# Tani843/Mixed_Precision_Multigrid_Solvers_for_PDEs

Hardware: AMD Instinct MI355X
Metric: MDoF/s per V-cycle on 2D Poisson (higher is better)
Workload: dtype f64 (adaptive policy); 1 GPU; 2D Poisson 4097^2 adaptive fp32->fp64 (switch_threshold=1e-6), V(2,2) weighted-Jacobi omega=0.8, 11 levels, 1xMI355X; levels=11, cycle=V(2,2), smoother=jacobi, parallelism=1 GPU

## Files before the change

### include/mghip.h

```cpp
#ifndef MGHIP_H
#define MGHIP_H

#include <stdint.h>

#ifdef __cplusplus
extern "C" {
#endif

#define MG_OK 0
#define MG_ERR_INVALID_VALUE (-1)
#define MG_ERR_NO_DEVICE (-2)
#define MG_ERR_HIP (-3)
#define MG_ERR_STATE (-4)
#define MG_ERR_ALLOC (-5)

typedef enum { MG_F32 = 0, MG_F64 = 1 } mg_dtype;
typedef enum {
  MG_JACOBI = 0,
  MG_RBGS = 1,
  MG_LEXGS = 2
} mg_smoother_t;
typedef enum { MG_CYCLE_V = 0, MG_CYCLE_W = 1, MG_CYCLE_F = 2 } mg_cycle_t;
typedef enum {
  MG_PREC_DOUBLE = 0,
// ... 16 lines not shown
  double coarse_tol;
  int32_t coarse_maxit;
  int32_t precision;
  double switch_threshold;
  double memory_threshold_gb;
  int32_t adaptive_reference_rule;
  int32_t device;
  int32_t profile;
  int32_t colour_offset;
  int32_t fused;
  int32_t tail;
  int32_t fmg_cycles;
  int32_t speculate;
  int32_t coarse_direct;
  int32_t mixed_split;
} mg_config;

typedef struct mg_stats {
  double solve_seconds;
  double h2d_seconds;
  double d2h_seconds;
  double initial_residual;
  int32_t precision_switches;
  int32_t last_coarse_sweeps;
  int32_t switch_reason;
  double fp32_floor;
} mg_stats;

typedef struct mg_handle mg_handle;

// ... 196 lines not shown
```

### mixed_precision_multigrid_solvers_for_pdes_amd/_build.py

```python
import os
import shutil
import subprocess
from concurrent.futures import ThreadPoolExecutor

HERE = os.path.dirname(os.path.abspath(__file__))
CSRC = os.path.join(HERE, "csrc")
LIBDIR = os.path.join(HERE, "lib")
OBJDIR = os.path.join(LIBDIR, "obj")
LIBPATH = os.path.join(LIBDIR, "libmghip.so")
SOURCES = [os.path.join(CSRC, n) for n in ("mg_launch.hip", "mg_engine.hip", "mg_solve.hip", "mg_dev.hip", "mg_plan.hip", "mg_tail.hip", "mg_pcg.hip", "mg_heat.hip")]
HEADERS = [os.path.join(CSRC, n) for n in ("mg_kernels.hpp", "mg_rb_kernels.hpp", "mg_tail_kernels.hpp", "mg_host.hpp", "mg_launch.hpp", "mg_pcg_kernels.hpp",
                                               "mg_heat_kernels.hpp")] + \
          [os.path.join(os.path.dirname(HERE), "include", n) for n in ("mghip.h", "mghip_heat.h")]
DEPS = SOURCES + HEADERS
_HOST_UNIT = ("mg_rb_kernels.hpp", "mg_tail_kernels.hpp", "mg_pcg_kernels.hpp", "mg_heat_kernels.hpp")
NOT_INCLUDED = {"mg_launch.hip": ("mg_tail_kernels.hpp", "mg_pcg_kernels.hpp", "mg_heat_kernels.hpp"),
                "mg_engine.hip": _HOST_UNIT, "mg_solve.hip": _HOST_UNIT, "mg_dev.hip": _HOST_UNIT,
                "mg_tail.hip": ("mg_launch.hpp", "mg_pcg_kernels.hpp", "mg_heat_kernels.hpp"),
                "mg_pcg.hip": ("mg_rb_kernels.hpp", "mg_tail_kernels.hpp", "mg_heat_kernels.hpp"),
                "mg_heat.hip": ("mg_rb_kernels.hpp", "mg_tail_kernels.hpp", "mg_launch.hpp", "mg_pcg_kernels.hpp"),
                "mg_plan.hip": ("mg_kernels.hpp", "mg_rb_kernels.hpp", "mg_tail_kernels.hpp", "mg_host.hpp", "mg_launch.hpp",
                                "mg_pcg_kernels.hpp", "mg_heat_kernels.hpp", "mghip_heat.h")}
FLAGS = ["--offload-arch=gfx950", "-O3", "-std=c++17", "-fPIC", "-ffp-contract=off", "-Wall", "-Wno-unused-function"]


def extra_flags():
    return os.environ.get("MGHIP_EXTRA_FLAGS", "").split()


def hipcc_path():
    for cand in (os.environ.get("HIPCC"), "/opt/rocm/bin/hipcc", shutil.which("hipcc")):
        if cand and os.path.exists(cand):
            return cand
    raise RuntimeError("hipcc not found (set HIPCC or install ROCm under /opt/rocm)")


def source_hash():
# ... 84 lines not shown
```

### mixed_precision_multigrid_solvers_for_pdes_amd/_lib.py

```python
import ctypes as C
import os

import numpy as np

from . import _build

MG_OK = 0
MG_ERR_INVALID_VALUE, MG_ERR_NO_DEVICE, MG_ERR_HIP, MG_ERR_STATE, MG_ERR_ALLOC, MG_ERR_TIMEOUT = -1, -2, -3, -4, -5, -6
MG_PLAN_PHASES = 7
PLAN_PHASE_NAMES = ("legs", "halo_copy", "halo_exchange", "coarse_allgather", "replicated_engine", "allreduce", "other")


class PlanTimeout(RuntimeError):
    """mg_plan_wait gave up (MG_ERR_TIMEOUT): the queued device work is still queued, so the process must not
    synchronise on it again -- report and leave (distributed.bench_main does, with os._exit)."""
MG_F32, MG_F64 = 0, 1
MG_JACOBI, MG_RBGS, MG_LEXGS = 0, 1, 2
MG_CYCLE_V, MG_CYCLE_W, MG_CYCLE_F = 0, 1, 2
MG_PREC_DOUBLE, MG_PREC_SINGLE, MG_PREC_MIXED_LEVELS, MG_PREC_ADAPTIVE, MG_PREC_SINGLE_MANAGED, MG_PREC_DEFECT = 0, 1, 2, 3, 4, 5

CYCLES = {"V": MG_CYCLE_V, "W": MG_CYCLE_W, "F": MG_CYCLE_F}


class MgConfig(C.Structure):
    _fields_ = [
        ("nx", C.c_int32), ("ny", C.c_int32),
        ("x0", C.c_double), ("x1", C.c_double), ("y0", C.c_double), ("y1", C.c_double),
        ("coeff", C.c_double),
        ("max_levels", C.c_int32), ("cycle", C.c_int32), ("pre", C.c_int32), ("post", C.c_int32),
        ("smoother", C.c_int32),
        ("omega", C.c_double),
        ("coarse_tol", C.c_double), ("coarse_maxit", C.c_int32),
        ("precision", C.c_int32),
        ("switch_threshold", C.c_double), ("memory_threshold_gb", C.c_double),
        ("adaptive_reference_rule", C.c_int32),
        ("device", C.c_int32), ("profile", C.c_int32), ("colour_offset", C.c_int32), ("fused", C.c_int32),
        ("tail", C.c_int32), ("fmg_cycles", C.c_int32), ("speculate", C.c_int32), ("coarse_direct", C.c_int32),
        ("mixed_split", C.c_int32),
    ]


class MgStats(C.Structure):
    _fields_ = [
        ("solve_seconds", C.c_double), ("h2d_seconds", C.c_double), ("d2h_seconds", C.c_double),
        ("initial_residual", C.c_double),
        ("precision_switches", C.c_int32), ("last_coarse_sweeps", C.c_int32),
        ("switch_reason", C.c_int32), ("fp32_floor", C.c_double),
    ]


class MgPcgStats(C.Structure):
    _fields_ = [("solve_seconds", C.c_double), ("precond_seconds", C.c_double), ("initial_residual", C.c_double),
                ("true_residual", C.c_double), ("iterations", C.c_int32), ("status", C.c_int32)]
# ... 239 lines not shown
```

### mixed_precision_multigrid_solvers_for_pdes_amd/csrc/mg_engine.hip

```cpp
#include "mg_launch.hpp"

#include <cstring>

namespace mgh {

std::string& last_error() {
  thread_local std::string msg;
  return msg;
}

static int upload(std::string* err, void* dev, int ddt, int ld, const void* host, int hdt, int nx, int ny, void* staging,
           hipStream_t st) {
  if (ddt == hdt) {
    HIPC(err, hipMemcpy2DAsync(dev, (size_t)ld * esize(ddt), host, (size_t)ny * esize(hdt), (size_t)ny * esize(hdt), nx,
                               hipMemcpyHostToDevice, st));
  } else {
    const int lds = pitch_elems(hdt, ny);
    HIPC(err, hipMemcpy2DAsync(staging, (size_t)lds * esize(hdt), host, (size_t)ny * esize(hdt), (size_t)ny * esize(hdt),
                               nx, hipMemcpyHostToDevice, st));
    d_convert(hdt, ddt, staging, dev, nx, ny, lds, ld, st);
  }
  HIPC(err, hipStreamSynchronize(st));
  return MG_OK;
}
// ... 170 lines not shown
    h->tail_start = k;
    break;
  }
  h->tail_direct = false;
  h->tail_minv_sigma = -1.0;
  if (h->tail_start < 0) return MG_OK;
  h->tail_direct = want_direct(h);
  std::vector<int> ops;
  tail_schedule(h, h->tail_start, h->tail_start, 2, ops);
  h->tail_nops = (int)ops.size();
  HIPC(&h->err, hipMalloc((void**)&h->d_tail_ops, sizeof(int) * ops.size()));
  HIPC(&h->err, hipMemcpy(h->d_tail_ops, ops.data(), sizeof(int) * ops.size(), hipMemcpyHostToDevice));
  if (tail_set_attrs(kTailPoolLimit + 1024) != MG_OK) h->tail_start = -1;
  return MG_OK;
}
static int plan_tail(mg_handle* h) {
  int rc = plan_tail_lds(h);
  if (rc != MG_OK) return rc;
  rc = tail2_plan(h);
  if (rc == MG_OK && h->tail2_start >= 0) h->tail_direct = want_direct(h);
  return rc;
}

static int build_coarse_inverse(mg_handle* h) {
  const Level& v = h->lv[h->L() - 1];
  const int cnx = v.nx, cny = v.ny, my = cny - 2, n = (cnx - 2) * my;
  if (n < 1 || n > 64) return fail(&h->err, MG_ERR_INVALID_VALUE, "coarse_direct: the coarsest grid has more than 64 unknowns");
  std::vector<double> a((size_t)cnx * cny, 1.0);
  if (h->varcoef) {
    const int dt = h->grid_dtype;
    std::vector<unsigned char> buf((size_t)cnx * v.ld[dt] * esize(dt));
    HIPC(&h->err, hipMemcpyAsync(buf.data(), v.a[dt], buf.size(), hipMemcpyDeviceToHost, h->stream));
    HIPC(&h->err, hipStreamSynchronize(h->stream));
    for (int i = 0; i < cnx; ++i)
      for (int j = 0; j < cny; ++j)
// ... 41 lines not shown
    HIPC(&h->err, hipMemcpy(h->d_minv, inv.data(), sizeof(double) * inv.size(), hipMemcpyHostToDevice));
    h->minv_n = n;
  }
  h->tail_minv_sigma = h->sigma;
  return MG_OK;
}

static void extra_sweeps(mg_handle* h, Level& f, int dt, LegGeom& g, int extra) {
  for (; extra > 0; extra -= g.nsweep) {
    g.nsweep = std::min(2, extra);
    d_sweeps(h->cfg.smoother, dt, f.u[dt], f.rhs[dt], f.t[dt], g, h->stream);
    std::swap(f.u[dt], f.t[dt]);
  }
}

int cycle_fused(mg_handle* h, int l, bool zero_u, int part) {
  const int L = h->L();
  Level& f = h->lv[l];
  const int dt = h->level_dtype(l);
  const size_t bytes = (size_t)f.nx * f.ld[dt] * esize(dt);
  const bool tail2 = l == h->tail2_start, tail_lds = l == h->tail_start && h->tail2_start < 0;
  if ((tail2 || tail_lds) && h->cfg.tail != 0) {
    if (h->tail_direct && h->tail_minv_sigma != h->sigma) { const int rc = build_coarse_inverse(h); if (rc != MG_OK) return rc; }
    if (tail2) return tail2_launch(h, zero_u);
    launch_tail(h, zero_u);
    return MG_OK;
  }
  if (l == L - 1) {
    coarse_solve(h, l, zero_u);
    return MG_OK;
  }
  Level& c = h->lv[l + 1];
  const int dc = h->level_dtype(l + 1);
  const bool fine = (l == 0);
  const int sm = h->cfg.smoother;
  LegGeom g = leg_geom(h, l, dt, dc);
  if (part != kPartBack) {
    StageTimer tm(h, &f, 0);
    if (h->cfg.pre > 2 && zero_u) { (void)hipMemsetAsync(f.u[dt], 0, bytes, h->stream); zero_u = false; }
    extra_sweeps(h, f, dt, g, h->cfg.pre - 2);
    g.nsweep = std::min(2, h->cfg.pre);
    d_down(sm, dt, dc, f.u[dt], f.rhs[dt], f.t[dt], c.rhs[dc], g, zero_u, h->stream);
    std::swap(f.u[dt], f.t[dt]);
  }
  for (int k = 0, n = h->visits(l); k < n && part != kPartBack; ++k) {
// ... 509 lines not shown
  HIPC(&h->err, hipSetDevice(h->cfg.device));
  for (int k = 0; k < ncycles; ++k) {
    const int rc = run_cycle(h);
    if (rc != MG_OK) return fail(&h->err, rc, "cycle: unsupported precision combination");
  }
  HIPC(&h->err, hipGetLastError());
  return MG_OK;
}

int mg_time_op(mg_handle* h, int op, int level, int dtype, int reps, double* avg_ms) {
  if (!h || !avg_ms || reps < 1 || level < 0 || level >= h->L() || !valid_dtype(dtype))
    return fail(h ? &h->err : nullptr, MG_ERR_INVALID_VALUE, "mg_time_op: bad argument");
  HIPC(&h->err, hipSetDevice(h->cfg.device));
  Level& v = h->lv[level];
  const int dt = dtype;
  if (op != 6 && (!v.u[dt] || !v.rhs[dt])) return fail(&h->err, MG_ERR_STATE, "mg_time_op: level has no arrays of that dtype");
  if ((op == 0 || op == 10) && h->cfg.smoother != MG_JACOBI) return fail(&h->err, MG_ERR_STATE, "mg_time_op: jacobi needs a Jacobi-configured handle");
  if ((op == 0 || (op >= 7 && op <= 9)) && !v.t[dt]) return fail(&h->err, MG_ERR_STATE, "mg_time_op: no ping-pong buffer on this level");
  if ((op == 2 || op == 4 || op == 5 || op == 7 || op == 8) && (level >= h->L() - 1 || !v.r[dt])) return fail(&h->err, MG_ERR_STATE, "mg_time_op: no coarser level");
  static const int exp_nsweep = exp_env("MG_EXP_NSWEEP", 2);
  h->norm_partials = 0;
  if (level == 0 && (op == 0 || op == 1 || (op >= 5 && op <= 9) || op == 12 || op == 13)) h->iterate_zero = false;
  std::vector<void*> hbm_sets;
  struct FreeSets { std::vector<void*>& v; ~FreeSets() { for (void* p : v) (void)hipFree(p); } } free_sets{hbm_sets};
  int nsets = 0, set_idx = 0;
  if (op == 10 || op == 11) {
    const size_t bytes = (size_t)v.nx * v.ld[dt] * esize(dt);
    nsets = std::max<int>(3, (int)((768ull << 20) / (3 * bytes)) + 1);
    for (int k = 0; k < 3 * nsets; ++k) {
      void* p = nullptr;
      HIPC(&h->err, hipMalloc(&p, bytes));
// ... 28 lines not shown
                  std::swap(v.u[dt], v.t[dt]); } break;
        case 8: { Level& c = h->lv[level + 1]; const int dc = c.u[dt] ? dt : 1 - dt;
                  LegGeom g = leg_geom(h, level, dt, dc); g.nsweep = exp_nsweep;
                  if (d_up(h->cfg.smoother, dt, dc, h->grid_dtype, v.u[dt], v.rhs[dt], v.t[dt], c.u[dc], h->partials, g, level == 0, h->stream) < 0) return MG_ERR_INVALID_VALUE;
                  std::swap(v.u[dt], v.t[dt]); } break;
        case 9: { LegGeom g = leg_geom(h, level, dt, -1); g.nsweep = exp_nsweep;
                  d_sweeps(h->cfg.smoother, dt, v.u[dt], v.rhs[dt], v.t[dt], g, h->stream);
                  std::swap(v.u[dt], v.t[dt]); } break;
        case 12: case 13: {
                  const int phase0 = h->phase;
                  if (h->cfg.precision == MG_PREC_ADAPTIVE) h->phase = dt;
                  const bool ok = level == 0 && span_ok(h) && h->level_dtype(0) == dt;
                  const int rc2 = ok ? cycle_span(h, op == 12) : MG_ERR_INVALID_VALUE;
                  h->phase = phase0;
                  if (rc2 != MG_OK) return rc2; } break;
        default: return MG_ERR_INVALID_VALUE;
      }
    }
    return MG_OK;
  };
  int rc = run(1);
  if (rc != MG_OK) { (void)hipEventDestroy(e0); (void)hipEventDestroy(e1); return fail(&h->err, rc, "mg_time_op: unsupported op"); }
  HIPC(&h->err, hipEventRecord(e0, h->stream));
  rc = run(reps);
  HIPC(&h->err, hipEventRecord(e1, h->stream));
  HIPC(&h->err, hipEventSynchronize(e1));
  float ms = 0;
  HIPC(&h->err, hipEventElapsedTime(&ms, e0, e1));
  (void)hipEventDestroy(e0); (void)hipEventDestroy(e1);
  *avg_ms = (double)ms / reps;
// ... 10 lines not shown
```

### mixed_precision_multigrid_solvers_for_pdes_amd/csrc/mg_host.hpp

```cpp
#pragma once

#include <hip/hip_runtime.h>

#include <algorithm>
#include <chrono>
#include <cmath>
#include <cstdlib>
#include <string>
#include <type_traits>
#include <vector>

#include "../../include/mghip.h"
#include "../../include/mghip_heat.h"
#include "mg_kernels.hpp"

namespace mgh {

std::string& last_error();
inline int fail(std::string* where, int code, const std::string& msg) {
  last_error() = msg;
  if (where) *where = msg;
  return code;
}
#define HIPC(errstr, call)                                                                         \
// ... 103 lines not shown
  bool have_rhs = false;
  bool varcoef = false;
  double sigma = 0.0;
  double rd_sigma = -1.0;
  double ring_sumsq[2] = {0, 0};
  unsigned rhs_gen = 1;
  unsigned rings_gen[2] = {0, 0};
  bool iterate_zero = false;
  unsigned zero_norm_gen[2] = {0, 0};
  double zero_norm_val[2] = {0, 0};
  int norm_partials = 0;
  int tail_start = -1;
  bool span_ring[2] = {false, false};
  int tail2_start = -1;
  int tail2_ntop = 0;
  int* d_tail_ops = nullptr;
  int tail_nops = 0;
  bool tail_direct = false;
  double tail_minv[81] = {0};
  double* d_minv = nullptr;
  int minv_n = 0;
  double tail_minv_sigma = -1.0;
  std::string err;
  std::vector<double> adapt_hist;

  int L() const { return (int)lv.size(); }
  int visits(int l) const {
    return cfg.cycle == MG_CYCLE_W ? 2 : cfg.cycle == MG_CYCLE_F ? std::max(1, 1 << std::max(0, L() - l - 2)) : 1;
  }
  int level_dtype_in(int l, int ph) const {
// ... 46 lines not shown
```

### mixed_precision_multigrid_solvers_for_pdes_amd/csrc/mg_launch.hpp

```cpp
#pragma once

#include "mg_host.hpp"

namespace mgh {

int pitch_elems(int dt, int ny);
size_t max_partials(int nx, int ny);

void d_jacobi(int dt, const void* u, const void* rhs, void* out, int nx, int ny, int ld, double hx, double hy,
              double omega, hipStream_t st, bool fine = false, double sigma = 0.0);
void d_rbgs_colour(int dt, void* u, const void* rhs, int nx, int ny, int ld, double hx, double hy, double omega,
                   int colour, int poff, hipStream_t st, bool fine = false, double sigma = 0.0);
void d_residual(int dt, const void* u, const void* f, void* r, int nx, int ny, int ld, double hx, double hy,
                double coeff, hipStream_t st, bool fine = false, double sigma = 0.0);
int d_residual_norm(int dt, const void* u, const void* f, double* partials, int nx, int ny, int ld, double hx,
                    double hy, double coeff, hipStream_t st, bool fine = false, double sigma = 0.0);
int d_sumsq(int dt, const void* x, double* partials, int ld, int i_lo, int i_hi, int j_lo, int j_hi, hipStream_t st);
void launch_reduce(const double* partials, int n, double* out, hipStream_t st, mg::HostMailbox* mailbox = nullptr,
                   unsigned long long seq = 0);
void d_restrict_sub(int di, int dout, const void* fine, void* coarse, int ldf, int nxc, int nyc, int ldc, int sides,
                    hipStream_t st);
void d_restrict(int di, int dout, const void* fine, void* coarse, int nxf, int nyf, int ldf, int ldc, hipStream_t st);
int d_prolong_sub(bool add, int dc, int df, int dcomp, const void* e, void* u, int nxf, int nyf, int ldf, int nxc, int nyc,
                  int ldc, int sides, hipStream_t st);
// ... 24 lines not shown
  double sigma = 0.0;
  const void* acoef = nullptr;
  const void* rdiag = nullptr;
  int rb = 0;
};
bool use_rb(const LegGeom& g);

int d_span(int dt, int dcomp, const void* u, const void* rhs, void* out_mid, void* out_next, const void* e_c, void* rhs_c,
           double* partials, const LegGeom& g, int nsweep_pre, hipStream_t st, int sm = MG_JACOBI);
void d_down(int sm, int dt, int dx, const void* u, const void* rhs, void* out, void* rhs_c, const LegGeom& g, bool zero_init,
            hipStream_t st);
int d_up(int sm, int dt, int dx, int dcomp, const void* u, const void* rhs, void* out, const void* e_c, double* partials,
         const LegGeom& g, bool norm, hipStream_t st);
void d_sweeps(int sm, int dt, const void* u, const void* rhs, void* out, const LegGeom& g, hipStream_t st);

constexpr size_t kTailPoolLimit = 150 * 1024;
size_t tail_pool_bytes(const mg_handle* h, int k, size_t esz, size_t esz_last);
int tail_set_attrs(size_t bytes);
void launch_tail(mg_handle* h, bool zero_top);

int launch_defect(mg_handle* h, bool update);
void d_stream_triad(int dt, const void* a, const void* b, void* out, int nx, int ny, int ld, hipStream_t st);
void d_residual_f32in_f64out(const float* u, const float* f, double* r, int nx, int ny, int ld_in, int ld_out, double hx,
                             double hy, double coeff, hipStream_t st);

}
```

### mixed_precision_multigrid_solvers_for_pdes_amd/engine.py

```python
import ctypes as C

import numpy as np

from . import _lib


def _direct_code(coarse_direct):
    import os
    if coarse_direct is None:
        coarse_direct = {"0": False, "1": True}.get(os.environ.get("MG_COARSE_DIRECT", "auto"), "auto")
    if isinstance(coarse_direct, str):
        if coarse_direct != "auto":
            raise ValueError(f"coarse_direct: True, False, 'auto' or None, not {coarse_direct!r}")
        return -1
    return int(bool(coarse_direct))


class MultigridEngine:

    def __init__(self, nx, ny, domain=(0.0, 1.0, 0.0, 1.0), coeff=-1.0, max_levels=4, cycle="V", pre=2, post=2,
                 smoother=_lib.MG_JACOBI, omega=0.8, coarse_tol=1e-12, coarse_maxit=1000,
                 precision=_lib.MG_PREC_DOUBLE, switch_threshold=1e-6, memory_threshold_gb=4.0,
                 adaptive_reference_rule=False, device=0, profile=False, colour_offset=0, fused=2, tail=True, speculate=True, fmg_cycles=0,
                 mixed_split=0, coarse_direct=None):
        lib = _lib.load()
        if isinstance(cycle, str):
            if cycle not in _lib.CYCLES:
                raise ValueError(f"unknown cycle type {cycle!r}")
            cycle = _lib.CYCLES[cycle]
        cfg = _lib.MgConfig(int(nx), int(ny), float(domain[0]), float(domain[1]), float(domain[2]), float(domain[3]),
                            float(coeff), int(max_levels), int(cycle), int(pre), int(post), int(smoother),
                            float(omega), float(coarse_tol), int(coarse_maxit), int(precision),
                            float(switch_threshold), float(memory_threshold_gb), int(bool(adaptive_reference_rule)),
                            int(device), int(bool(profile)), int(colour_offset), int(fused), int(tail), int(fmg_cycles), (2 if speculate is True else int(speculate)),
                            _direct_code(coarse_direct), int(mixed_split))
        self.cfg = cfg
        self._h = C.c_void_p(None)
        _lib.check(lib.mg_create(C.byref(cfg), C.byref(self._h)))
        self._lib = lib
        n = C.c_int(0)
        self._check(lib.mg_num_levels(self._h, C.byref(n)))
        self.num_levels = n.value
        self.shapes = []
        for l in range(self.num_levels):
            a, b = C.c_int(0), C.c_int(0)
            self._check(lib.mg_level_shape(self._h, l, C.byref(a), C.byref(b)))
            self.shapes.append((a.value, b.value))
        self.nx, self.ny = int(nx), int(ny)

    def _check(self, rc):
# ... 122 lines not shown
        self._check(self._lib.mg_get_solution_device(self._h, *self._dev_args(t)))

    def set_stream(self, stream):
        if stream is None:
            self._check(self._lib.mg_set_stream(self._h, None, 1))
        else:
            self._check(self._lib.mg_set_stream(self._h, stream if isinstance(stream, C.c_void_p) else C.c_void_p(int(stream)), 0))

    def get_stream(self):
        out = C.c_void_p(None)
        self._check(self._lib.mg_get_stream(self._h, C.byref(out)))
        return out.value or 0

    def time_op(self, op, level=0, dtype=np.float64, reps=20):
        ops = {"jacobi": 0, "rbgs": 1, "residual": 2, "residual_norm": 3, "restrict": 4, "prolong": 5, "cycle": 6,
               "down_leg": 7, "up_leg": 8, "sweeps2": 9, "jacobi_hbm": 10, "stream_hbm": 11, "span_leg": 12, "span_leg_nomid": 13}
        out = C.c_double(0.0)
        self._check(self._lib.mg_time_op(self._h, ops[op] if isinstance(op, str) else int(op), int(level),
                                         _lib.dtype_code(dtype), int(reps), C.byref(out)))
        return out.value

    def level_timings(self):
        res = {}
        for l in range(self.num_levels):
            t = (C.c_double * 3)()
            self._check(self._lib.mg_level_timings(self._h, l, t))
            res[l] = {"smooth_time": t[0], "restrict_time": t[1], "prolong_time": t[2]}
        return res
```

Measured before the change: 81550 MDoF/s.

## Merge two or three mid-size multigrid levels into single down and up kernels

Adds merged down and up kernels that process a group of up to three mid-size levels (at most 520 per side, just above the LDS tail) in one launch each. Each block keeps an overlapping halo region in LDS and runs the smoothing sweeps, residual and full-weighting restriction through all grouped levels, then on the way up does prolongation plus post-smoothing. This is meant to cut kernel launches and the global-memory round trips between levels. The cost is redundant halo computation and large LDS use at 512 threads per block, which may limit occupancy. It is enabled by default through MG_MERGE=1 for V-cycle Jacobi.

```diff
diff --git a/include/mghip.h b/include/mghip.h
--- a/include/mghip.h
+++ b/include/mghip.h
@@ -54,6 +54,7 @@
   int32_t speculate;
   int32_t coarse_direct;
   int32_t mixed_split;
+  int32_t merge;
 } mg_config;
 
 typedef struct mg_stats {
diff --git a/mixed_precision_multigrid_solvers_for_pdes_amd/_build.py b/mixed_precision_multigrid_solvers_for_pdes_amd/_build.py
--- a/mixed_precision_multigrid_solvers_for_pdes_amd/_build.py
+++ b/mixed_precision_multigrid_solvers_for_pdes_amd/_build.py
@@ -8,19 +8,21 @@
 LIBDIR = os.path.join(HERE, "lib")
 OBJDIR = os.path.join(LIBDIR, "obj")
 LIBPATH = os.path.join(LIBDIR, "libmghip.so")
-SOURCES = [os.path.join(CSRC, n) for n in ("mg_launch.hip", "mg_engine.hip", "mg_solve.hip", "mg_dev.hip", "mg_plan.hip", "mg_tail.hip", "mg_pcg.hip", "mg_heat.hip")]
+SOURCES = [os.path.join(CSRC, n) for n in ("mg_launch.hip", "mg_engine.hip", "mg_solve.hip", "mg_dev.hip", "mg_plan.hip", "mg_tail.hip", "mg_pcg.hip", "mg_heat.hip", "mg_merge.hip")]
 HEADERS = [os.path.join(CSRC, n) for n in ("mg_kernels.hpp", "mg_rb_kernels.hpp", "mg_tail_kernels.hpp", "mg_host.hpp", "mg_launch.hpp", "mg_pcg_kernels.hpp",
-                                               "mg_heat_kernels.hpp")] + \
+                                               "mg_heat_kernels.hpp", "mg_merge_kernels.hpp", "mg_merge_geom.hpp")] + \
           [os.path.join(os.path.dirname(HERE), "include", n) for n in ("mghip.h", "mghip_heat.h")]
 DEPS = SOURCES + HEADERS
-_HOST_UNIT = ("mg_rb_kernels.hpp", "mg_tail_kernels.hpp", "mg_pcg_kernels.hpp", "mg_heat_kernels.hpp")
-NOT_INCLUDED = {"mg_launch.hip": ("mg_tail_kernels.hpp", "mg_pcg_kernels.hpp", "mg_heat_kernels.hpp"),
+_MERGE = ("mg_merge_kernels.hpp", "mg_merge_geom.hpp")
+_HOST_UNIT = ("mg_rb_kernels.hpp", "mg_tail_kernels.hpp", "mg_pcg_kernels.hpp", "mg_heat_kernels.hpp") + _MERGE
+NOT_INCLUDED = {"mg_launch.hip": ("mg_tail_kernels.hpp", "mg_pcg_kernels.hpp", "mg_heat_kernels.hpp") + _MERGE,
+                "mg_merge.hip": ("mg_rb_kernels.hpp", "mg_tail_kernels.hpp", "mg_pcg_kernels.hpp", "mg_heat_kernels.hpp"),
                 "mg_engine.hip": _HOST_UNIT, "mg_solve.hip": _HOST_UNIT, "mg_dev.hip": _HOST_UNIT,
-                "mg_tail.hip": ("mg_launch.hpp", "mg_pcg_kernels.hpp", "mg_heat_kernels.hpp"),
-                "mg_pcg.hip": ("mg_rb_kernels.hpp", "mg_tail_kernels.hpp", "mg_heat_kernels.hpp"),
-                "mg_heat.hip": ("mg_rb_kernels.hpp", "mg_tail_kernels.hpp", "mg_launch.hpp", "mg_pcg_kernels.hpp"),
+                "mg_tail.hip": ("mg_launch.hpp", "mg_pcg_kernels.hpp", "mg_heat_kernels.hpp") + _MERGE,
+                "mg_pcg.hip": ("mg_rb_kernels.hpp", "mg_tail_kernels.hpp", "mg_heat_kernels.hpp") + _MERGE,
+                "mg_heat.hip": ("mg_rb_kernels.hpp", "mg_tail_kernels.hpp", "mg_launch.hpp", "mg_pcg_kernels.hpp") + _MERGE,
                 "mg_plan.hip": ("mg_kernels.hpp", "mg_rb_kernels.hpp", "mg_tail_kernels.hpp", "mg_host.hpp", "mg_launch.hpp",
-                                "mg_pcg_kernels.hpp", "mg_heat_kernels.hpp", "mghip_heat.h")}
+                                "mg_pcg_kernels.hpp", "mg_heat_kernels.hpp", "mghip_heat.h") + _MERGE}
 FLAGS = ["--offload-arch=gfx950", "-O3", "-std=c++17", "-fPIC", "-ffp-contract=off", "-Wall", "-Wno-unused-function"]
 
 
diff --git a/mixed_precision_multigrid_solvers_for_pdes_amd/_lib.py b/mixed_precision_multigrid_solvers_for_pdes_amd/_lib.py
--- a/mixed_precision_multigrid_solvers_for_pdes_amd/_lib.py
+++ b/mixed_precision_multigrid_solvers_for_pdes_amd/_lib.py
@@ -36,7 +36,7 @@
         ("adaptive_reference_rule", C.c_int32),
         ("device", C.c_int32), ("profile", C.c_int32), ("colour_offset", C.c_int32), ("fused", C.c_int32),
         ("tail", C.c_int32), ("fmg_cycles", C.c_int32), ("speculate", C.c_int32), ("coarse_direct", C.c_int32),
-        ("mixed_split", C.c_int32),
+        ("mixed_split", C.c_int32), ("merge", C.c_int32),
     ]
 
 
diff --git a/mixed_precision_multigrid_solvers_for_pdes_amd/csrc/mg_engine.hip b/mixed_precision_multigrid_solvers_for_pdes_amd/csrc/mg_engine.hip
--- a/mixed_precision_multigrid_solvers_for_pdes_amd/csrc/mg_engine.hip
+++ b/mixed_precision_multigrid_solvers_for_pdes_amd/csrc/mg_engine.hip
@@ -208,11 +208,25 @@
   if (tail_set_attrs(kTailPoolLimit + 1024) != MG_OK) h->tail_start = -1;
   return MG_OK;
 }
+static void plan_merge(mg_handle* h) {
+  h->merge_l0 = -1;
+  h->merge_nl = 0;
+  const int tail = h->tail2_start >= 0 ? h->tail2_start : h->tail_start;
+  if (tail < 0) return;
+  int first = tail;
+  while (first > 1 && std::max(h->lv[first - 1].nx, h->lv[first - 1].ny) <= 520) --first;
+  static const int max_nl = exp_env("MG_EXP_MERGE_NL", 3);
+  const int nl = std::min(std::min(3, max_nl), tail - first);
+  if (nl < 2) return;
+  h->merge_l0 = tail - nl;
+  h->merge_nl = nl;
+}
 static int plan_tail(mg_handle* h) {
   int rc = plan_tail_lds(h);
   if (rc != MG_OK) return rc;
   rc = tail2_plan(h);
   if (rc == MG_OK && h->tail2_start >= 0) h->tail_direct = want_direct(h);
+  plan_merge(h);
   return rc;
 }
 
@@ -284,6 +298,53 @@
   }
 }
 
+static MergeDesc merge_desc(const mg_handle* h, int dt, int nsweep) {
+  MergeDesc m;
+  m.nl = h->merge_nl;
+  for (int k = 0; k < m.nl; ++k) {
+    const Level& v = h->lv[h->merge_l0 + k];
+    MergeLevelDesc& d = m.lv[k];
+    d.u_in = v.u[dt]; d.u_out = v.t[dt]; d.rhs = v.rhs[dt];
+    d.nx = v.nx; d.ny = v.ny; d.ld = v.ld[dt]; d.hx = v.hx; d.hy = v.hy;
+  }
+  m.ldc = h->lv[h->merge_l0 + m.nl].ld[dt];
+  m.nsweep = nsweep; m.omega = h->cfg.omega; m.coeff = h->cfg.coeff; m.sigma = h->sigma;
+  return m;
+}
+static bool merge_arrays(const mg_handle* h, int dt) {
+  if (h->merge_l0 < 0) return false;
+  for (int l = h->merge_l0; l < h->merge_l0 + h->merge_nl; ++l)
+    if (!h->lv[l].u[dt] || !h->lv[l].t[dt] || !h->lv[l].rhs[dt]) return false;
+  const Level& c = h->lv[h->merge_l0 + h->merge_nl];
+  return c.u[dt] && c.rhs[dt];
+}
+static bool merge_ok(const mg_handle* h, int l, bool zero_u, int part) {
+  if (h->cfg.merge != 1 || l != h->merge_l0 || !zero_u || part != kPartFull || h->cfg.tail == 0) return false;
+  if (h->cfg.cycle != MG_CYCLE_V || h->cfg.smoother != MG_JACOBI || h->varcoef || h->cfg.profile) return false;
+  if (h->cfg.pre < 1 || h->cfg.pre > 2 || h->cfg.post < 1 || h->cfg.post > 2) return false;
+  const int dt = h->level_dtype(l);
+  for (int k = 1; k <= h->merge_nl; ++k)
+    if (h->level_dtype(l + k) != dt) return false;
+  if (dt == MG_F64 && h->grid_dtype == MG_F32) return false;
+  return merge_arrays(h, dt);
+}
+static void merge_swap(mg_handle* h, int dt) {
+  for (int l = h->merge_l0; l < h->merge_l0 + h->merge_nl; ++l) std::swap(h->lv[l].u[dt], h->lv[l].t[dt]);
+}
+static void down_merged(mg_handle* h, int dt, int nsweep) {
+  MergeDesc m = merge_desc(h, dt, nsweep);
+  m.coarse = h->lv[h->merge_l0 + h->merge_nl].rhs[dt];
+  d_down_merged(dt, m, h->stream);
+  merge_swap(h, dt);
+}
+static int up_merged(mg_handle* h, int dt, int nsweep) {
+  MergeDesc m = merge_desc(h, dt, nsweep);
+  m.coarse = h->lv[h->merge_l0 + h->merge_nl].u[dt];
+  if (d_up_merged(dt, h->grid_dtype, m, h->stream) < 0) return MG_ERR_INVALID_VALUE;
+  merge_swap(h, dt);
+  return MG_OK;
+}
+
 int cycle_fused(mg_handle* h, int l, bool zero_u, int part) {
   const int L = h->L();
   Level& f = h->lv[l];
@@ -299,6 +360,11 @@
   if (l == L - 1) {
     coarse_solve(h, l, zero_u);
     return MG_OK;
+  }
+  if (merge_ok(h, l, zero_u, part)) {
+    down_merged(h, dt, h->cfg.pre);
+    const int rc = cycle_fused(h, l + h->merge_nl, true);
+    return rc != MG_OK ? rc : up_merged(h, dt, h->cfg.post);
   }
   Level& c = h->lv[l + 1];
   const int dc = h->level_dtype(l + 1);
@@ -838,7 +904,10 @@
   HIPC(&h->err, hipSetDevice(h->cfg.device));
   Level& v = h->lv[level];
   const int dt = dtype;
-  if (op != 6 && (!v.u[dt] || !v.rhs[dt])) return fail(&h->err, MG_ERR_STATE, "mg_time_op: level has no arrays of that dtype");
+  if ((op == 14 || op == 15) && (!merge_arrays(h, dt) || level < h->merge_l0 || level >= h->merge_l0 + h->merge_nl || h->varcoef ||
+                                 (dt == MG_F64 && h->grid_dtype == MG_F32)))
+    return fail(&h->err, MG_ERR_STATE, "mg_time_op: no merged legs here (the level is in no group of levels, or not in that dtype)");
+  if (op != 6 && op != 14 && op != 15 && (!v.u[dt] || !v.rhs[dt])) return fail(&h->err, MG_ERR_STATE, "mg_time_op: level has no arrays of that dtype");
   if ((op == 0 || op == 10) && h->cfg.smoother != MG_JACOBI) return fail(&h->err, MG_ERR_STATE, "mg_time_op: jacobi needs a Jacobi-configured handle");
   if ((op == 0 || (op >= 7 && op <= 9)) && !v.t[dt]) return fail(&h->err, MG_ERR_STATE, "mg_time_op: no ping-pong buffer on this level");
   if ((op == 2 || op == 4 || op == 5 || op == 7 || op == 8) && (level >= h->L() - 1 || !v.r[dt])) return fail(&h->err, MG_ERR_STATE, "mg_time_op: no coarser level");
@@ -897,6 +966,8 @@
                   const int rc2 = ok ? cycle_span(h, op == 12) : MG_ERR_INVALID_VALUE;
                   h->phase = phase0;
                   if (rc2 != MG_OK) return rc2; } break;
+        case 14: down_merged(h, dt, exp_nsweep); break;
+        case 15: { const int rc2 = up_merged(h, dt, exp_nsweep); if (rc2 != MG_OK) return rc2; } break;
         default: return MG_ERR_INVALID_VALUE;
       }
     }
diff --git a/mixed_precision_multigrid_solvers_for_pdes_amd/csrc/mg_host.hpp b/mixed_precision_multigrid_solvers_for_pdes_amd/csrc/mg_host.hpp
--- a/mixed_precision_multigrid_solvers_for_pdes_amd/csrc/mg_host.hpp
+++ b/mixed_precision_multigrid_solvers_for_pdes_amd/csrc/mg_host.hpp
@@ -141,6 +141,8 @@
   bool span_ring[2] = {false, false};
   int tail2_start = -1;
   int tail2_ntop = 0;
+  int merge_l0 = -1;
+  int merge_nl = 0;
   int* d_tail_ops = nullptr;
   int tail_nops = 0;
   bool tail_direct = false;
diff --git a/mixed_precision_multigrid_solvers_for_pdes_amd/csrc/mg_launch.hpp b/mixed_precision_multigrid_solvers_for_pdes_amd/csrc/mg_launch.hpp
--- a/mixed_precision_multigrid_solvers_for_pdes_amd/csrc/mg_launch.hpp
+++ b/mixed_precision_multigrid_solvers_for_pdes_amd/csrc/mg_launch.hpp
@@ -62,6 +62,23 @@
          const LegGeom& g, bool norm, hipStream_t st);
 void d_sweeps(int sm, int dt, const void* u, const void* rhs, void* out, const LegGeom& g, hipStream_t st);
 
+struct MergeLevelDesc {
+  const void* u_in = nullptr;
+  void* u_out = nullptr;
+  void* rhs = nullptr;
+  int nx = 0, ny = 0, ld = 0;
+  double hx = 0, hy = 0;
+};
+struct MergeDesc {
+  MergeLevelDesc lv[3];
+  int nl = 0;
+  void* coarse = nullptr;
+  int ldc = 0, nsweep = 0;
+  double omega = 0, coeff = 0, sigma = 0;
+};
+void d_down_merged(int dt, const MergeDesc& m, hipStream_t st);
+int d_up_merged(int dt, int dcomp, const MergeDesc& m, hipStream_t st);
+
 constexpr size_t kTailPoolLimit = 150 * 1024;
 size_t tail_pool_bytes(const mg_handle* h, int k, size_t esz, size_t esz_last);
 int tail_set_attrs(size_t bytes);
diff --git a/mixed_precision_multigrid_solvers_for_pdes_amd/csrc/mg_merge.hip b/mixed_precision_multigrid_solvers_for_pdes_amd/csrc/mg_merge.hip
--- /dev/null
+++ b/mixed_precision_multigrid_solvers_for_pdes_amd/csrc/mg_merge.hip
@@ -0,0 +1,83 @@
+#include "mg_launch.hpp"
+#include "mg_merge_kernels.hpp"
+
+namespace mgh {
+
+constexpr int kDownBI = 4, kDownBJ = 4;
+constexpr int kUpBI = 32, kUpBJ = 32;
+
+template <typename T>
+static mg::MergeArgs<T> merge_args(const MergeDesc& m) {
+  mg::MergeArgs<T> a;
+  for (int k = 0; k < m.nl; ++k) {
+    const MergeLevelDesc& d = m.lv[k];
+    const Coef c = coefs(d.hx, d.hy, m.sigma);
+    mg::MergeLevel<T>& L = a.lv[k];
+    L.u_in = (const T*)d.u_in; L.u_out = (T*)d.u_out; L.rhs = (T*)d.rhs;
+    L.nx = d.nx; L.ny = d.ny; L.ld = d.ld; L.use_div = c.pow2 ? 0 : 1;
+    L.ihx2 = (T)c.ihx2; L.ihy2 = (T)c.ihy2; L.invD = (T)c.invD; L.D = (T)c.diag;
+  }
+  for (int k = m.nl; k < mgm::kMaxNL; ++k) a.lv[k] = a.lv[m.nl - 1];
+  a.coarse = (T*)m.coarse; a.ldc = m.ldc; a.nsweep = m.nsweep; a.nbj = 0;
+  a.omega = (T)m.omega; a.one_m_omega = (T)(1.0 - m.omega); a.coeff = (T)m.coeff;
+  return a;
+}
+
+template <typename T, int NL, int BI, int BJ>
+static void launch_down(const MergeDesc& m, hipStream_t st) {
+  mg::MergeArgs<T> a = merge_args<T>(m);
+  const int nbi = mgm::blocks(mgm::level_n(m.lv[0].nx, NL), BI);
+  a.nbj = mgm::blocks(mgm::level_n(m.lv[0].ny, NL), BJ);
+  hipLaunchKernelGGL((mg::merged_down_kernel<T, NL, BI, BJ>), dim3(nbi * a.nbj), dim3(mgm::kBlock), 0, st, a);
+}
+template <typename T, typename TC, int NL, int BI, int BJ>
+static void launch_up(const MergeDesc& m, hipStream_t st) {
+  mg::MergeArgs<T> a = merge_args<T>(m);
+  const int nbi = mgm::blocks(m.lv[0].nx, BI);
+  a.nbj = mgm::blocks(m.lv[0].ny, BJ);
+  hipLaunchKernelGGL((mg::merged_up_kernel<T, TC, NL, BI, BJ>), dim3(nbi * a.nbj), dim3(mgm::kBlock), 0, st, a);
+}
+
+template <typename T, int NL>
+static void down_shaped(const MergeDesc& m, hipStream_t st) {
+#ifdef MG_EXPERIMENTS
+  static const int shape = exp_env("MG_EXP_MERGE_DOWN", 0);
+  if (shape == 1) return launch_down<T, NL, 8, 8>(m, st);
+  if (shape == 2) return launch_down<T, NL, 4, 16>(m, st);
+  if (shape == 3) return launch_down<T, NL, 4, 8>(m, st);
+  if (shape == 4) return launch_down<T, NL, 2, 8>(m, st);
+#endif
+  launch_down<T, NL, kDownBI, kDownBJ>(m, st);
+}
+template <typename T, typename TC, int NL>
+static void up_shaped(const MergeDesc& m, hipStream_t st) {
+#ifdef MG_EXPERIMENTS
+  static const int shape = exp_env("MG_EXP_MERGE_UP", 0);
+  if (shape == 1) return launch_up<T, TC, NL, 64, 64>(m, st);
+  if (shape == 2) return launch_up<T, TC, NL, 32, 64>(m, st);
+  if (shape == 3) return launch_up<T, TC, NL, 16, 64>(m, st);
+  if (shape == 4) return launch_up<T, TC, NL, 16, 32>(m, st);
+#endif
+  launch_up<T, TC, NL, kUpBI, kUpBJ>(m, st);
+}
+
+void d_down_merged(int dt, const MergeDesc& m, hipStream_t st) {
+  with_dtype(dt, [&](auto t) {
+    using T = decltype(t);
+    if (m.nl == 3) down_shaped<T, 3>(m, st);
+    else down_shaped<T, 2>(m, st);
+  });
+}
+int d_up_merged(int dt, int dcomp, const MergeDesc& m, hipStream_t st) {
+  return with_dtype(dt, dcomp, [&](auto t, auto tc) {
+    using T = decltype(t); using TC = decltype(tc);
+    if constexpr (!interp_ok<T, T, TC>) return -1;
+    else {
+      if (m.nl == 3) up_shaped<T, TC, 3>(m, st);
+      else up_shaped<T, TC, 2>(m, st);
+      return 0;
+    }
+  });
+}
+
+}
diff --git a/mixed_precision_multigrid_solvers_for_pdes_amd/csrc/mg_merge_geom.hpp b/mixed_precision_multigrid_solvers_for_pdes_amd/csrc/mg_merge_geom.hpp
--- /dev/null
+++ b/mixed_precision_multigrid_solvers_for_pdes_amd/csrc/mg_merge_geom.hpp
@@ -0,0 +1,132 @@
+#pragma once
+
+#if defined(__HIPCC__)
+#define MGM_HD __host__ __device__ __forceinline__
+#else
+#define MGM_HD inline
+#endif
+
+namespace mgm {
+
+constexpr int kMaxNL = 3;
+constexpr int kMaxSweeps = 2;
+constexpr int kBlock = 512;
+constexpr int kLdsLimit = 160 * 1024;
+
+struct Iv { int lo, hi; };
+struct Box { Iv i, j; };
+
+MGM_HD int imin(int a, int b) { return a < b ? a : b; }
+MGM_HD int imax(int a, int b) { return a > b ? a : b; }
+MGM_HD int size(Iv a) { return a.hi > a.lo ? a.hi - a.lo : 0; }
+MGM_HD Iv grow(Iv a, int k) { return Iv{a.lo - k, a.hi + k}; }
+MGM_HD Iv interior(Iv a, int n) { return Iv{imax(a.lo, 1), imin(a.hi, n - 1)}; }
+MGM_HD bool has(Iv a, int x) { return x >= a.lo && x < a.hi; }
+MGM_HD bool has(const Box& b, int i, int j) { return has(b.i, i) && has(b.j, j); }
+MGM_HD bool inside(Iv in, Iv out) { return size(in) == 0 || (in.lo >= out.lo && in.hi <= out.hi); }
+MGM_HD int level_n(int n0, int k) { return ((n0 - 1) >> k) + 1; }
+MGM_HD int blocks(int n, int B) { return (n - 2 + B - 1) / B; }
+
+template <int NL> struct Down1 {
+  Iv out;
+  Iv resid[NL];
+  Iv rhs[NL];
+  Iv own[NL + 1];
+  int org[NL];
+};
+MGM_HD Iv down_sweep(Iv resid, int n, int pre, int s) { return interior(grow(resid, 1 + pre - s), n); }
+template <int NL, int B> MGM_HD Down1<NL> down_1d(int n0, int pre, int b) {
+  Down1<NL> g;
+  const int nout = level_n(n0, NL);
+  g.out = Iv{imin(1 + b * B, nout - 1), imin(1 + (b + 1) * B, nout - 1)};
+  const bool last = g.out.hi == nout - 1;
+  g.own[NL] = g.out;
+  Iv need = g.out;
+  for (int k = NL - 1; k >= 0; --k) {
+    const int n = level_n(n0, k), m = NL - k;
+    g.resid[k] = Iv{2 * need.lo - 1, 2 * need.hi};
+    g.rhs[k] = down_sweep(g.resid[k], n, pre, 1);
+    g.org[k] = g.resid[k].lo - pre - 1;
+    g.own[k] = Iv{imin(((g.out.lo - 1) << m) + 1, n - 1), last ? n - 1 : imin(((g.out.hi - 1) << m) + 1, n - 1)};
+    need = g.rhs[k];
+  }
+  return g;
+}
+constexpr int down_rhs_dim(int B, int NL, int k) { return k == NL ? B : 2 * down_rhs_dim(B, NL, k + 1) + 1 + 2 * kMaxSweeps; }
+constexpr int down_region_dim(int B, int NL, int k) { return down_rhs_dim(B, NL, k) + 2; }
+
+template <int NL> struct DownGeom {
+  Down1<NL> i, j;
+  MGM_HD Box out() const { return Box{i.out, j.out}; }
+  MGM_HD Box resid(int k) const { return Box{i.resid[k], j.resid[k]}; }
+  MGM_HD Box rhs(int k) const { return Box{i.rhs[k], j.rhs[k]}; }
+  MGM_HD Box own(int k) const { return Box{i.own[k], j.own[k]}; }
+};
+MGM_HD Box down_sweep_box(Box resid, int nx, int ny, int pre, int s) {
+  return Box{down_sweep(resid.i, nx, pre, s), down_sweep(resid.j, ny, pre, s)};
+}
+template <int NL, int BI, int BJ> MGM_HD DownGeom<NL> down_geom(int nx0, int ny0, int pre, int bi, int bj) {
+  return DownGeom<NL>{down_1d<NL, BI>(nx0, pre, bi), down_1d<NL, BJ>(ny0, pre, bj)};
+}
+
+template <int NL> struct Up1 {
+  Iv want[NL + 1];
+  Iv fin[NL];
+  Iv interp[NL];
+  Iv own[NL];
+  int org[NL];
+};
+MGM_HD Iv up_sweep(Iv fin, int n, int post, int s) { return interior(grow(fin, post - s), n); }
+template <int NL, int B> MGM_HD Up1<NL> up_1d(int n0, int post, int b) {
+  Up1<NL> g;
+  g.want[0] = Iv{imin(1 + b * B, n0 - 1), imin(1 + (b + 1) * B, n0 - 1)};
+  for (int k = 0; k < NL; ++k) {
+    const int n = level_n(n0, k), Bk = B >> k;
+    g.own[k] = Iv{imin(1 + b * Bk, n - 1), imin(1 + (b + 1) * Bk, n - 1)};
+    g.fin[k] = interior(g.want[k], n);
+    g.interp[k] = up_sweep(g.fin[k], n, post, 0);
+    g.org[k] = g.fin[k].lo - post;
+    g.want[k + 1] = size(g.interp[k]) == 0 ? Iv{0, 0} : Iv{g.interp[k].lo >> 1, (g.interp[k].hi >> 1) + 1};
+  }
+  return g;
+}
+constexpr int up_want_dim(int B, int k) { return k == 0 ? B : (up_want_dim(B, k - 1) + 2 * kMaxSweeps) / 2 + 2; }
+constexpr int up_region_dim(int B, int k) { return up_want_dim(B, k) + 2 * kMaxSweeps; }
+
+template <int NL> struct UpGeom {
+  Up1<NL> i, j;
+  MGM_HD Box want(int k) const { return Box{i.want[k], j.want[k]}; }
+  MGM_HD Box fin(int k) const { return Box{i.fin[k], j.fin[k]}; }
+  MGM_HD Box interp(int k) const { return Box{i.interp[k], j.interp[k]}; }
+  MGM_HD Box own(int k) const { return Box{i.own[k], j.own[k]}; }
+};
+MGM_HD Box up_sweep_box(Box fin, int nx, int ny, int post, int s) {
+  return Box{up_sweep(fin.i, nx, post, s), up_sweep(fin.j, ny, post, s)};
+}
+template <int NL, int BI, int BJ> MGM_HD UpGeom<NL> up_geom(int nx0, int ny0, int post, int bi, int bj) {
+  return UpGeom<NL>{up_1d<NL, BI>(nx0, post, bi), up_1d<NL, BJ>(ny0, post, bj)};
+}
+
+template <int NL, int BI, int BJ> struct DownShape {
+  static constexpr int ri(int k) { return down_region_dim(BI, NL, k); }
+  static constexpr int rj(int k) { return down_region_dim(BJ, NL, k); }
+  static constexpr int elems(int k) { return ri(k) * rj(k); }
+  static constexpr int off(int k) { return k == 0 ? 0 : off(k - 1) + ((elems(k - 1) + 1) & ~1); }
+  static constexpr int total() { return off(NL); }
+  static constexpr int cpt(int k) { return (elems(k) + kBlock - 1) / kBlock; }
+  static constexpr int out_cpt() { return (BI * BJ + kBlock - 1) / kBlock; }
+};
+template <int NL, int BI, int BJ> struct UpShape {
+  static_assert(BI % (1 << (NL - 1)) == 0 && BJ % (1 << (NL - 1)) == 0, "owned blocks of the coarser levels need whole cells");
+  static constexpr int ri(int k) { return up_region_dim(BI, k); }
+  static constexpr int rj(int k) { return up_region_dim(BJ, k); }
+  static constexpr int elems(int k) { return ri(k) * rj(k); }
+  static constexpr int pi() { return up_want_dim(BI, NL); }
+  static constexpr int pj() { return up_want_dim(BJ, NL); }
+  static constexpr int off(int k) { return k == 0 ? 0 : off(k - 1) + ((elems(k - 1) + 1) & ~1); }
+  static constexpr int total() { return off(NL) + pi() * pj(); }
+  static constexpr int cpt(int k) { return (elems(k) + kBlock - 1) / kBlock; }
+  static constexpr int patch_cpt() { return (pi() * pj() + kBlock - 1) / kBlock; }
+};
+
+}
diff --git a/mixed_precision_multigrid_solvers_for_pdes_amd/csrc/mg_merge_kernels.hpp b/mixed_precision_multigrid_solvers_for_pdes_amd/csrc/mg_merge_kernels.hpp
--- /dev/null
+++ b/mixed_precision_multigrid_solvers_for_pdes_amd/csrc/mg_merge_kernels.hpp
@@ -0,0 +1,248 @@
+#pragma once
+
+#include "mg_kernels.hpp"
+#include "mg_merge_geom.hpp"
+
+namespace mg {
+
+template <typename T> struct MergeLevel {
+  const T* u_in;
+  T* u_out;
+  T* rhs;
+  int nx, ny, ld;
+  int use_div;
+  T ihx2, ihy2, invD, D;
+};
+template <typename T> struct MergeArgs {
+  MergeLevel<T> lv[mgm::kMaxNL];
+  T* coarse;
+  int ldc;
+  int nsweep;
+  int nbj;
+  T omega, one_m_omega, coeff;
+};
+
+template <typename T>
+__device__ __forceinline__ T merge_jacobi(const MergeLevel<T>& L, T omega, T one_m_omega, T f, T up, T dn, T w, T ea, T mid) {
+  const T nb = L.ihx2 * (dn + up) + L.ihy2 * (ea + w);
+  const T un = L.use_div ? (f + nb) / L.D : (f + nb) * L.invD;
+  return one_m_omega * mid + omega * un;
+}
+template <typename T>
+__device__ __forceinline__ T merge_residual(const MergeLevel<T>& L, T coeff, T f, T up, T dn, T w, T ea, T mid) {
+  const T au = coeff * (((dn + up) * L.ihx2 + (ea + w) * L.ihy2) - mid * L.D);
+  return f - au;
+}
+template <typename T> __device__ __forceinline__ T merge_full_weighting(const T* p, int stride) {
+  const T corners = ((p[-stride - 1] + p[-stride + 1]) + p[stride - 1]) + p[stride + 1];
+  const T edges = ((p[-stride] + p[stride]) + p[-1]) + p[1];
+  return (T(1.0 / 16.0) * corners + T(1.0 / 8.0) * edges) + T(1.0 / 4.0) * p[0];
+}
+template <typename T, typename TC>
+__device__ __forceinline__ TC merge_prolong(const T* e, int stride, int gi, int gj) {
+  const T* p = e + (gi >> 1) * stride + (gj >> 1);
+  if (gi & 1) {
+    if (gj & 1) return TC(0.25) * ((((TC)p[0] + (TC)p[1]) + (TC)p[stride]) + (TC)p[stride + 1]);
+    return TC(0.5) * ((TC)p[0] + (TC)p[stride]);
+  }
+  if (gj & 1) return TC(0.5) * ((TC)p[0] + (TC)p[1]);
+  return (TC)p[0];
+}
+
+template <int RJ, int ELEMS, int CPT, typename T>
+__device__ __forceinline__ void merge_sweep(T* s, T (&v)[CPT], const T (&f)[CPT], const mgm::Box& box, int oi, int oj,
+                                            const MergeLevel<T>& L, T omega, T one_m_omega) {
+#pragma unroll
+  for (int c = 0; c < CPT; ++c) {
+    const int idx = threadIdx.x + c * mgm::kBlock, li = idx / RJ, lj = idx - li * RJ;
+    if (idx < ELEMS && mgm::has(box, oi + li, oj + lj))
+      v[c] = merge_jacobi(L, omega, one_m_omega, f[c], s[idx - RJ], s[idx + RJ], s[idx - 1], s[idx + 1], v[c]);
+  }
+  __syncthreads();
+#pragma unroll
+  for (int c = 0; c < CPT; ++c) {
+    const int idx = threadIdx.x + c * mgm::kBlock, li = idx / RJ, lj = idx - li * RJ;
+    if (idx < ELEMS && mgm::has(box, oi + li, oj + lj)) s[idx] = v[c];
+  }
+  __syncthreads();
+}
+template <int RJ, int ELEMS, int CPT, typename T>
+__device__ __forceinline__ void merge_store_owned(T* out, int ld, const T (&v)[CPT], const mgm::Box& own, int oi, int oj) {
+#pragma unroll
+  for (int c = 0; c < CPT; ++c) {
+    const int idx = threadIdx.x + c * mgm::kBlock, li = idx / RJ, lj = idx - li * RJ;
+    if (idx < ELEMS && mgm::has(own, oi + li, oj + lj)) out[(size_t)(oi + li) * ld + (oj + lj)] = v[c];
+  }
+}
+
+template <typename T, int NL, int BI, int BJ, int K, int CPT>
+__device__ __forceinline__ void merged_down_level(T* lds, const MergeArgs<T>& a, const mgm::DownGeom<NL>& g, const T (&f)[CPT]) {
+  using S = mgm::DownShape<NL, BI, BJ>;
+  constexpr int RJ = S::rj(K), ELEMS = S::elems(K), OFF = S::off(K);
+  static_assert(CPT == S::cpt(K), "register tile of another level");
+  T* s = lds + OFF;
+  const MergeLevel<T>& L = a.lv[K];
+  const int oi = g.i.org[K], oj = g.j.org[K], pre = a.nsweep;
+  const mgm::Box resid = g.resid(K);
+  if (K > 0) merge_store_owned<RJ, ELEMS, CPT>(L.rhs, L.ld, f, g.own(K), oi, oj);
+  T v[CPT];
+  {
+    const mgm::Box box = mgm::down_sweep_box(resid, L.nx, L.ny, pre, 1);
+#pragma unroll
+    for (int c = 0; c < CPT; ++c) {
+      const int idx = threadIdx.x + c * mgm::kBlock, li = idx / RJ, lj = idx - li * RJ;
+      v[c] = T(0);
+      if (idx < ELEMS) {
+        if (mgm::has(box, oi + li, oj + lj)) v[c] = merge_jacobi(L, a.omega, a.one_m_omega, f[c], T(0), T(0), T(0), T(0), T(0));
+        s[idx] = v[c];
+      }
+    }
+    __syncthreads();
+  }
+  for (int sw = 2; sw <= pre; ++sw)
+    merge_sweep<RJ, ELEMS, CPT>(s, v, f, mgm::down_sweep_box(resid, L.nx, L.ny, pre, sw), oi, oj, L, a.omega, a.one_m_omega);
+  merge_store_owned<RJ, ELEMS, CPT>(L.u_out, L.ld, v, g.own(K), oi, oj);
+#pragma unroll
+  for (int c = 0; c < CPT; ++c) {
+    const int idx = threadIdx.x + c * mgm::kBlock, li = idx / RJ, lj = idx - li * RJ;
+    if (idx < ELEMS && mgm::has(resid, oi + li, oj + lj))
+      v[c] = merge_residual(L, a.coeff, f[c], s[idx - RJ], s[idx + RJ], s[idx - 1], s[idx + 1], v[c]);
+  }
+  __syncthreads();
+#pragma unroll
+  for (int c = 0; c < CPT; ++c) {
+    const int idx = threadIdx.x + c * mgm::kBlock, li = idx / RJ, lj = idx - li * RJ;
+    if (idx < ELEMS && mgm::has(resid, oi + li, oj + lj)) s[idx] = v[c];
+  }
+  __syncthreads();
+  if constexpr (K + 1 < NL) {
+    constexpr int RJ2 = S::rj(K + 1), ELEMS2 = S::elems(K + 1), CPT2 = S::cpt(K + 1);
+    const int oi2 = g.i.org[K + 1], oj2 = g.j.org[K + 1];
+    const mgm::Box need = g.rhs(K + 1);
+    T f2[CPT2];
+#pragma unroll
+    for (int c = 0; c < CPT2; ++c) {
+      const int idx = threadIdx.x + c * mgm::kBlock, li = idx / RJ2, lj = idx - li * RJ2;
+      const int ic = oi2 + li, jc = oj2 + lj;
+      f2[c] = T(0);
+      if (idx < ELEMS2 && mgm::has(need, ic, jc)) f2[c] = merge_full_weighting(s + (2 * ic - oi) * RJ + (2 * jc - oj), RJ);
+    }
+    merged_down_level<T, NL, BI, BJ, K + 1, CPT2>(lds, a, g, f2);
+  } else {
+    const mgm::Box out = g.out();
+    const int wj = mgm::size(out.j), n = mgm::size(out.i) * wj;
+    for (int idx = threadIdx.x; idx < n; idx += mgm::kBlock) {
+      const int ic = out.i.lo + idx / wj, jc = out.j.lo + idx % wj;
+      a.coarse[(size_t)ic * a.ldc + jc] = merge_full_weighting(s + (2 * ic - oi) * RJ + (2 * jc - oj), RJ);
+    }
+  }
+}
+
+template <typename T, int NL, int BI, int BJ>
+__global__ __launch_bounds__(mgm::kBlock) void merged_down_kernel(MergeArgs<T> a) {
+  using S = mgm::DownShape<NL, BI, BJ>;
+  constexpr int TOTAL = S::total();
+  static_assert((size_t)TOTAL * sizeof(T) <= (size_t)mgm::kLdsLimit, "regions do not fit the LDS");
+  __shared__ __attribute__((aligned(16))) T lds[TOTAL];
+  const int bi = blockIdx.x / a.nbj, bj = blockIdx.x - bi * a.nbj;
+  const mgm::DownGeom<NL> g = mgm::down_geom<NL, BI, BJ>(a.lv[0].nx, a.lv[0].ny, a.nsweep, bi, bj);
+  constexpr int RJ = S::rj(0), ELEMS = S::elems(0), CPT = S::cpt(0);
+  const MergeLevel<T>& L = a.lv[0];
+  const mgm::Box box = g.rhs(0);
+  T f[CPT];
+#pragma unroll
+  for (int c = 0; c < CPT; ++c) {
+    const int idx = threadIdx.x + c * mgm::kBlock, li = idx / RJ, lj = idx - li * RJ;
+    const int gi = g.i.org[0] + li, gj = g.j.org[0] + lj;
+    f[c] = T(0);
+    if (idx < ELEMS && mgm::has(box, gi, gj)) f[c] = L.rhs[(size_t)gi * L.ld + gj];
+  }
+  merged_down_level<T, NL, BI, BJ, 0, CPT>(lds, a, g, f);
+}
+
+template <typename T, int CPT> struct MergeRegs { T u[CPT], f[CPT]; };
+
+template <typename T, int NL, int BI, int BJ, int K, int CPT>
+__device__ __forceinline__ void merged_up_load(const MergeArgs<T>& a, const mgm::UpGeom<NL>& g, MergeRegs<T, CPT>& r) {
+  using S = mgm::UpShape<NL, BI, BJ>;
+  constexpr int RJ = S::rj(K), ELEMS = S::elems(K);
+  const MergeLevel<T>& L = a.lv[K];
+  const mgm::Box bu = g.interp(K), bf = mgm::up_sweep_box(g.fin(K), L.nx, L.ny, a.nsweep, 1);
+#pragma unroll
+  for (int c = 0; c < CPT; ++c) {
+    const int idx = threadIdx.x + c * mgm::kBlock, li = idx / RJ, lj = idx - li * RJ;
+    const int gi = g.i.org[K] + li, gj = g.j.org[K] + lj;
+    r.u[c] = T(0);
+    r.f[c] = T(0);
+    if (idx < ELEMS && mgm::has(bu, gi, gj)) r.u[c] = L.u_in[(size_t)gi * L.ld + gj];
+    if (idx < ELEMS && mgm::has(bf, gi, gj)) r.f[c] = L.rhs[(size_t)gi * L.ld + gj];
+  }
+}
+template <typename T, typename TC, int NL, int BI, int BJ, int K, int CPT>
+__device__ __forceinline__ void merged_up_level(T* lds, const MergeArgs<T>& a, const mgm::UpGeom<NL>& g, MergeRegs<T, CPT>& r,
+                                                const T* e, int ei, int ej, int es) {
+  using S = mgm::UpShape<NL, BI, BJ>;
+  using TS = typename std::conditional<(sizeof(TC) > sizeof(T)), TC, T>::type;
+  constexpr int RJ = S::rj(K), ELEMS = S::elems(K), OFF = S::off(K);
+  T* s = lds + OFF;
+  const MergeLevel<T>& L = a.lv[K];
+  const int oi = g.i.org[K], oj = g.j.org[K], post = a.nsweep;
+  const mgm::Box bu = g.interp(K), fin = g.fin(K);
+  const T* e0 = e - ((ptrdiff_t)ei * es + ej);
+#pragma unroll
+  for (int c = 0; c < CPT; ++c) {
+    const int idx = threadIdx.x + c * mgm::kBlock, li = idx / RJ, lj = idx - li * RJ;
+    const int gi = oi + li, gj = oj + lj;
+    if (idx < ELEMS) {
+      if (mgm::has(bu, gi, gj)) r.u[c] = (T)((TS)r.u[c] + (TS)merge_prolong<T, TC>(e0, es, gi, gj));
+      s[idx] = r.u[c];
+    }
+  }
+  __syncthreads();
+  for (int sw = 1; sw <= post; ++sw)
+    merge_sweep<RJ, ELEMS, CPT>(s, r.u, r.f, mgm::up_sweep_box(fin, L.nx, L.ny, post, sw), oi, oj, L, a.omega, a.one_m_omega);
+  merge_store_owned<RJ, ELEMS, CPT>(L.u_out, L.ld, r.u, g.own(K), oi, oj);
+}
+
+template <typename T, typename TC, int NL, int BI, int BJ>
+__global__ __launch_bounds__(mgm::kBlock) void merged_up_kernel(MergeArgs<T> a) {
+  using S = mgm::UpShape<NL, BI, BJ>;
+  static_assert(NL == 2 || NL == 3, "groups of two or three levels");
+  constexpr int TOTAL = S::total(), PCPT = S::patch_cpt(), OFF1 = S::off(1), OFF2 = S::off(2), OFFP = S::off(NL);
+  constexpr int RJ1 = S::rj(1), RJ2 = S::rj(2);
+  static_assert((size_t)TOTAL * sizeof(T) <= (size_t)mgm::kLdsLimit, "regions do not fit the LDS");
+  __shared__ __attribute__((aligned(16))) T lds[TOTAL];
+  const int bi = blockIdx.x / a.nbj, bj = blockIdx.x - bi * a.nbj;
+  const mgm::UpGeom<NL> g = mgm::up_geom<NL, BI, BJ>(a.lv[0].nx, a.lv[0].ny, a.nsweep, bi, bj);
+  const mgm::Box pb = g.want(NL);
+  const int pw = mgm::size(pb.j), pn = mgm::size(pb.i) * pw;
+  T pv[PCPT];
+#pragma unroll
+  for (int c = 0; c < PCPT; ++c) {
+    const int idx = threadIdx.x + c * mgm::kBlock;
+    pv[c] = T(0);
+    if (idx < pn) pv[c] = a.coarse[(size_t)(pb.i.lo + idx / pw) * a.ldc + (pb.j.lo + idx % pw)];
+  }
+  MergeRegs<T, S::cpt(0)> r0;
+  MergeRegs<T, S::cpt(1)> r1;
+  MergeRegs<T, S::cpt(NL - 1)> r2;
+  merged_up_load<T, NL, BI, BJ, 0>(a, g, r0);
+  merged_up_load<T, NL, BI, BJ, 1>(a, g, r1);
+  if constexpr (NL == 3) merged_up_load<T, NL, BI, BJ, 2>(a, g, r2);
+  T* patch = lds + OFFP;
+#pragma unroll
+  for (int c = 0; c < PCPT; ++c) {
+    const int idx = threadIdx.x + c * mgm::kBlock;
+    if (idx < pn) patch[idx] = pv[c];
+  }
+  __syncthreads();
+  if constexpr (NL == 3) {
+    merged_up_level<T, TC, NL, BI, BJ, 2>(lds, a, g, r2, patch, pb.i.lo, pb.j.lo, pw);
+    merged_up_level<T, TC, NL, BI, BJ, 1>(lds, a, g, r1, lds + OFF2, g.i.org[2], g.j.org[2], RJ2);
+  } else {
+    merged_up_level<T, TC, NL, BI, BJ, 1>(lds, a, g, r1, patch, pb.i.lo, pb.j.lo, pw);
+  }
+  merged_up_level<T, TC, NL, BI, BJ, 0>(lds, a, g, r0, lds + OFF1, g.i.org[1], g.j.org[1], RJ1);
+}
+
+}
diff --git a/mixed_precision_multigrid_solvers_for_pdes_amd/engine.py b/mixed_precision_multigrid_solvers_for_pdes_amd/engine.py
--- a/mixed_precision_multigrid_solvers_for_pdes_amd/engine.py
+++ b/mixed_precision_multigrid_solvers_for_pdes_amd/engine.py
@@ -16,13 +16,22 @@
     return int(bool(coarse_direct))
 
 
+def _merge_code(merge):
+    import os
+    if merge is None:
+        merge = os.environ.get("MG_MERGE", "1")
+        if merge not in ("0", "1"):
+            raise ValueError(f"MG_MERGE: 0 or 1, not {merge!r}")
+    return int(bool(int(merge)))
+
+
 class MultigridEngine:
 
     def __init__(self, nx, ny, domain=(0.0, 1.0, 0.0, 1.0), coeff=-1.0, max_levels=4, cycle="V", pre=2, post=2,
                  smoother=_lib.MG_JACOBI, omega=0.8, coarse_tol=1e-12, coarse_maxit=1000,
                  precision=_lib.MG_PREC_DOUBLE, switch_threshold=1e-6, memory_threshold_gb=4.0,
                  adaptive_reference_rule=False, device=0, profile=False, colour_offset=0, fused=2, tail=True, speculate=True, fmg_cycles=0,
-                 mixed_split=0, coarse_direct=None):
+                 mixed_split=0, coarse_direct=None, merge=None):
         lib = _lib.load()
         if isinstance(cycle, str):
             if cycle not in _lib.CYCLES:
@@ -33,7 +42,7 @@
                             float(omega), float(coarse_tol), int(coarse_maxit), int(precision),
                             float(switch_threshold), float(memory_threshold_gb), int(bool(adaptive_reference_rule)),
                             int(device), int(bool(profile)), int(colour_offset), int(fused), int(tail), int(fmg_cycles), (2 if speculate is True else int(speculate)),
-                            _direct_code(coarse_direct), int(mixed_split))
+                            _direct_code(coarse_direct), int(mixed_split), _merge_code(merge))
         self.cfg = cfg
         self._h = C.c_void_p(None)
         _lib.check(lib.mg_create(C.byref(cfg), C.byref(self._h)))
@@ -186,7 +195,8 @@
 
     def time_op(self, op, level=0, dtype=np.float64, reps=20):
         ops = {"jacobi": 0, "rbgs": 1, "residual": 2, "residual_norm": 3, "restrict": 4, "prolong": 5, "cycle": 6,
-               "down_leg": 7, "up_leg": 8, "sweeps2": 9, "jacobi_hbm": 10, "stream_hbm": 11, "span_leg": 12, "span_leg_nomid": 13}
+               "down_leg": 7, "up_leg": 8, "sweeps2": 9, "jacobi_hbm": 10, "stream_hbm": 11, "span_leg": 12, "span_leg_nomid": 13,
+               "down_merged": 14, "up_merged": 15}
         out = C.c_double(0.0)
         self._check(self._lib.mg_time_op(self._h, ops[op] if isinstance(op, str) else int(op), int(level),
                                          _lib.dtype_code(dtype), int(reps), C.byref(out)))
```

Result: no change. 81570 MDoF/s (median of 3 runs) (+0.0%).
